# ChaissonLab/LRA

Measured on AMD Instinct MI355X. Metric: aligned Gbp/s, 30 kb ONT vs GRCh38 (MapRead_lowacc end to end incl. SAM text), per job, higher is better.
Workload: dtype int32

## Files before the change

lra_amd/csrc/aog.hip:

```cpp
#include "common.h"
#include <stdlib.h>
#include <algorithm>
#include <vector>
#include <type_traits>

namespace {

constexpr int MISS = -(1 << 30);
enum { A_DONE = 0, A_LEFT = 1, A_DOWN = 2, A_DIAG = 3, A_BORDER = 4, A_GAPLEFT = 5, A_GAPDOWN = 6 };

constexpr int CLASS_A_BYTES = 10 * 1024;
constexpr int CLASS_B_BYTES = 64 * 1024;
constexpr int CLASS_M1_BYTES = 20 * 1024;
constexpr int CLASS_M2_BYTES = 32 * 1024;
constexpr int LN_MAX = 24, LN_ROWW = 2;
constexpr int LN_ARROW_WORDS = LN_MAX * LN_ROWW, LN_PREV_WORDS = LN_MAX + 2, LN_CODE_BYTES = LN_MAX + 1;
constexpr int LN_BYTES = 64 * (4 * LN_ARROW_WORDS + 4 * LN_PREV_WORDS + 2 * LN_CODE_BYTES);
constexpr int NCLS = 19;
constexpr int CLASS_S_BYTES = 2560;

__device__ __forceinline__ int code_n(unsigned char c) {
  if (c < 8) return c & 3;
  switch (c) {
    case 'A': case 'a': return 0;
    case 'C': case 'c': return 1;
    case 'G': case 'g': return 2;
    case 'T': case 't': return 3;
    default: return 4;
  }
}

struct Geo {
  int qLen, tLen, diag, k, R, qB, tB;
  bool top;
  int n;
  int nUsed;
};

__device__ __forceinline__ bool make_geo(int qLen, int tLen, int k0, Geo& g) {
  g.qLen = qLen; g.tLen = tLen;
  g.diag = max(1, min(qLen, tLen));
  int k = min(g.diag, k0);
  g.top = true;
  if (g.diag + 2 * k >= max(qLen, tLen)) { k *= 2; g.top = false; }
  g.k = k;
  g.R = 2 * k + 3;
  long n = (long)(3 + k + g.diag) * g.R;
  g.qB = min(g.diag + k, qLen + 1);
  g.tB = min(g.diag + k, tLen + 1);
  if (n > (1L << 28)) { g.n = 0; g.nUsed = 0; return false; }
  g.n = (int)n;
  g.nUsed = g.top ? g.n : min(g.n, g.tB * g.R);
  return true;
}

__host__ __device__ __forceinline__ long align4(long x) { return (x + 3) & ~3L; }

__device__ __forceinline__ long need_bytes(const Geo& g) {
  long suf = g.top ? (4L * g.n + align4(g.n)) : 0;
  return 4L * g.nUsed + align4(g.nUsed) + suf + 16L * (g.diag + 1) + align4(g.qLen + 1) + align4(g.tLen + 1);
}

struct Work {
  int* sPre; int* sSuf; int* loMax; int* loIdx; int* upMax; int* upIdx;
  signed char* pPre; signed char* pSuf; unsigned char* qc; unsigned char* tc;
};

template <typename BytePtr>
__device__ __forceinline__ Work carve(BytePtr base, const Geo& g) {
  Work w;
  auto* p = base;
  w.sPre = (int*)p; p += 4L * g.nUsed;
  w.sSuf = (int*)p; if (g.top) p += 4L * g.n;
  w.loMax = (int*)p; p += 4L * (g.diag + 1);
  w.loIdx = (int*)p; p += 4L * (g.diag + 1);
  w.upMax = (int*)p; p += 4L * (g.diag + 1);
  w.upIdx = (int*)p; p += 4L * (g.diag + 1);
  w.pPre = (signed char*)p; p += align4(g.nUsed);
  w.pSuf = (signed char*)p; if (g.top) p += align4(g.n);
  w.qc = (unsigned char*)p; p += align4(g.qLen + 1);
  w.tc = (unsigned char*)p;
  return w;
}

__device__ __forceinline__ void wave_sync() {
  __builtin_amdgcn_fence(__ATOMIC_RELEASE, "workgroup");
  __builtin_amdgcn_wave_barrier();
  __builtin_amdgcn_fence(__ATOMIC_ACQUIRE, "workgroup");
}

__device__ __forceinline__ void wave_sync_lds() {
  __builtin_amdgcn_fence(__ATOMIC_RELEASE, "wavefront");
  __builtin_amdgcn_wave_barrier();
  __builtin_amdgcn_fence(__ATOMIC_ACQUIRE, "wavefront");
}

struct Problem {
  const char* q; const char* t;
  int qLen, tLen, k0, m, mm, indel;
};

__device__ __forceinline__ int dpp_from_prev_lane(int v) { return __builtin_amdgcn_update_dpp(MISS, v, 0x138, 0xf, 0xf, false); }
__device__ __forceinline__ int dpp_from_next_lane(int v) { return __builtin_amdgcn_update_dpp(MISS, v, 0x130, 0xf, 0xf, false); }

template <int G, typename ArrowPtr, typename CodePtr>
__device__ __forceinline__ int reg_fill(int lane, int gbase, const Geo& g, int m, int mm, int indel, ArrowPtr P, CodePtr qc, CodePtr tc) {
  const int qLen = g.qLen, tLen = g.tLen, k = g.k, R = g.R, diag = g.diag, qB = g.qB, tB = g.tB;
  auto pre = [&](int i, int j) -> int {
    int v = MISS;
    if (j == 0 && i >= 1 && i < k + 1) v = indel * i;
    if (i == 0 && j >= 1 && j <= k + 1) v = indel * j;
    if (i == 0 && j == 0) v = 0;
    if (qLen >= tLen) { if (j == i + k + 1 && i <= diag - k - 1) v = MISS; if (i == j + k + 1 && j >= 1 && j < diag + k - 1) v = MISS; }
    if (qLen <= tLen) { if (i == j + k + 1 && j < diag - 1) v = MISS; if (j == i + k + 1 && j >= 1 && j < diag + k) v = MISS; }
    return v;
  };
  const int Wd = 2 * k + 3;
  const int sLast = max((qB - 1) + (tB - 1), 0);
  const int ci = qB - 1, cj = tB - 1;
  int vE = MISS, vO = MISS;
  const bool firstE = ((0 - k - 1) & 1) == 0;
  const int dE = 2 * lane - k - 1, dO = dE + 1;
  const bool okE = 2 * lane < Wd && dE >= -k && dE <= k, okO = 2 * lane + 1 < Wd && dO >= -k && dO <= k;
  const int sLoE = okE ? 2 + abs(dE) : INT_MAX, sHiE = min(2 * (qB - 1) - dE, 2 * (tB - 1) + dE);
  const int sLoO = okO ? 2 + abs(dO) : INT_MAX, sHiO = min(2 * (qB - 1) - dO, 2 * (tB - 1) + dO);
  const int s0E = firstE ? 0 : 1, s0O = firstE ? 1 : 0;
  int iE = (s0E + dE) >> 1, jE = s0E - iE, iO = (s0O + dO) >> 1, jO = s0O - iO;
  int adE = jE * R + 2 * lane, adO = jO * R + 2 * lane + 1;
  auto codes_match = [&](int i, int j) -> bool { return qc[min(max(i, 0), qLen)] == tc[min(max(j, 0), tLen)]; };
  bool eqE = codes_match(iE, jE), eqO = codes_match(iO, jO);
  auto step = [&](int s, auto isE) {
    constexpr bool E = decltype(isE)::value;
    const int nb1 = E ? dpp_from_prev_lane(vO) : dpp_from_next_lane(vE);
    const int i = E ? iE : iO, j = E ? jE : jO;
    const bool nxt = codes_match(i + 1, j + 1);
    int v = MISS;
    if (s >= (E ? sLoE : sLoO) && s <= (E ? sHiE : sHiO)) {
      const int sIns = (E ? nb1 : vE) + indel;
      const int sDel = (E ? vO : nb1) + indel;
      const int sMat = (E ? vE : vO) + ((E ? eqE : eqO) ? m : mm);
      const int best = max(sIns, max(sDel, sMat));
      v = best;
      P[E ? adE : adO] = (signed char)((best == sIns) ? A_LEFT : (best == sDel) ? A_DOWN : A_DIAG);
    } else if (s <= k + 1) {
      if (2 * lane + (E ? 0 : 1) < Wd && i >= 0 && j >= 0) v = pre(i, j);
    }
    if (E) { vE = v; eqE = nxt; iE++; jE++; adE += R; } else { vO = v; eqO = nxt; iO++; jO++; adO += R; }
  };
  int s = 0;
  bool lastE;
  if (firstE) {
    for (; s + 1 <= sLast; s += 2) { step(s, std::true_type{}); step(s + 1, std::false_type{}); }
    lastE = false;
    if (s <= sLast) { step(s, std::true_type{}); lastE = true; }
  } else {
    for (; s + 1 <= sLast; s += 2) { step(s, std::false_type{}); step(s + 1, std::true_type{}); }
    lastE = true;
    if (s <= sLast) { step(s, std::false_type{}); lastE = false; }
  }
  const int ddc = ci - cj + k + 1;
  const int corner = lastE ? vE : vO;
  return (ci >= 0 && cj >= 0 && ddc >= 0 && ddc < Wd && ((ddc & 1) == 0) == lastE) ? __shfl(corner, gbase + (ddc >> 1)) : MISS;
}

template <int G, typename BytePtr>
__device__ __forceinline__ void solve(int wlane, const Problem& pr, const Geo& g, BytePtr mem, int* out_score,
                      int* out_nb, int* blocks, long cap, int* out_status, int* roll = nullptr, int chunkBytes = 8192) {
  const int qLen = g.qLen, tLen = g.tLen, k = g.k, R = g.R, diag = g.diag, n = g.n, nUsed = g.nUsed;
  const int m = pr.m, mm = pr.mm, indel = pr.indel;
  const int lane = wlane & (G - 1), gbase = wlane - lane;
  Work w = carve(mem, g);
  int status = 0;
  auto PI = [&](int i, int j) { return j * R + (i - j) + k + 1; };
  auto inb = [&](int s) { return s >= 0 && s < n; };
#define PSET(slot, sc, ar)                                                         \
  do { int s__ = (slot); if (inb(s__)) { if (s__ < nUsed) { if (!rolling) w.sPre[s__] = (sc); w.pPre[s__] = (ar); } } else status |= LRA_ST_OOB_SLOT; } while (0)
#define SSET(slot, sc, ar)                                                         \
  do { int s__ = (slot); if (inb(s__)) { w.sSuf[s__] = (sc); w.pSuf[s__] = (ar); } else status |= LRA_ST_OOB_SLOT; } while (0)

  for (int x = lane; x <= qLen; x += G) w.qc[x] = x ? code_n((unsigned char)pr.q[x - 1]) : 0;
  for (int x = lane; x <= tLen; x += G) w.tc[x] = x ? code_n((unsigned char)pr.t[x - 1]) : 0;
  const bool codesInLds = qLen + tLen + 2 <= 4096;
  const bool rolling = roll != nullptr && !g.top && (k + 2 <= G || (2 * k + 3 <= 256 && codesInLds));
  unsigned char* lq = (unsigned char*)(roll + 768); unsigned char* lt = lq + (qLen + 1);
  if (rolling && codesInLds) {
    for (int x = lane; x <= qLen; x += G) lq[x] = x ? code_n((unsigned char)pr.q[x - 1]) : 0;
    for (int x = lane; x <= tLen; x += G) lt[x] = x ? code_n((unsigned char)pr.t[x - 1]) : 0;
  }
  if (rolling) {
    const long head = min((long)nUsed, (long)((16 - ((uintptr_t)&w.pPre[0] & 15)) & 15));
    for (long x = lane; x < head; x += G) w.pPre[x] = -1;
    const long body = (nUsed - head) >> 4;
    int4* p16 = (int4*)(&w.pPre[0] + head);
    for (long x = lane; x < body; x += G) p16[x] = make_int4(-1, -1, -1, -1);
    for (long x = head + (body << 4) + lane; x < nUsed; x += G) w.pPre[x] = -1;
  }
  else for (int x = lane; x < nUsed; x += G) { w.sPre[x] = MISS; w.pPre[x] = -1; }
  if (g.top)
    for (int x = lane; x < n; x += G) { w.sSuf[x] = MISS; w.pSuf[x] = -1; }
  for (int x = lane; x <= diag; x += G) { w.loMax[x] = MISS; w.loIdx[x] = 0; w.upMax[x] = MISS; w.upIdx[x] = 0; }
  wave_sync();
  for (int i = 1 + lane; i < k + 1; i += G) PSET(PI(i, 0), indel * i, A_LEFT);
  for (int j = 1 + lane; j <= k + 1; j += G) PSET(PI(0, j), indel * j, A_DOWN);
  if (lane == 0) PSET(PI(0, 0), 0, A_DONE);
  wave_sync();
  if (qLen >= tLen) {
    for (int i = lane; i <= diag - k - 1; i += G) PSET(PI(i, i + k + 1), MISS, A_BORDER);
    for (int i = 1 + lane; i < diag + k - 1; i += G) PSET(PI(i + k + 1, i), MISS, A_BORDER);
  }
  if (qLen <= tLen) {
    for (int j = lane; j < diag - 1; j += G) PSET(PI(j + k + 1, j), MISS, A_BORDER);
    for (int j = 1 + lane; j < diag + k; j += G) PSET(PI(j - k - 1, j), MISS, A_BORDER);
  }
  wave_sync();
  const int qB = g.qB, tB = g.tB;
  int rollResult = MISS;
  if (rolling) {
    auto pre = [&](int i, int j) -> int {
      int v = MISS;
      if (j == 0 && i >= 1 && i < k + 1) v = indel * i;
      if (i == 0 && j >= 1 && j <= k + 1) v = indel * j;
      if (i == 0 && j == 0) v = 0;
      if (qLen >= tLen) { if (j == i + k + 1 && i <= diag - k - 1) v = MISS; if (i == j + k + 1 && j >= 1 && j < diag + k - 1) v = MISS; }
      if (qLen <= tLen) { if (i == j + k + 1 && j < diag - 1) v = MISS; if (j == i + k + 1 && j >= 1 && j < diag + k) v = MISS; }
      return v;
    };
    const int Wd = 2 * k + 3;
    const int sLast = (qB - 1) + (tB - 1);
    const bool inRegs = k + 2 <= G;
    if (inRegs) rollResult = codesInLds ? reg_fill<G>(lane, gbase, g, m, mm, indel, w.pPre, lq, lt) : reg_fill<G>(lane, gbase, g, m, mm, indel, w.pPre, w.qc, w.tc);
    for (int s = 0; !inRegs && s <= max(sLast, 0); s++) {
      int* cur = roll + (s % 3) * 256; const int* p1 = roll + ((s + 2) % 3) * 256; const int* p2 = roll + ((s + 1) % 3) * 256;
      int jlo = max(1, max(s - qB + 1, (s - k + 1) >> 1));
      if (s - k < 0) jlo = max(1, s - qB + 1);
      const int jhi = min(tB - 1, min(s - 1, (s + k) >> 1));
      for (int dd = lane; dd < Wd; dd += G) {
        const int d = dd - k - 1;
        int v = MISS;
        if (((s + d) & 1) == 0) {
          const int i = (s + d) >> 1, j = s - i;
          if (i >= 0 && j >= 0) {
            if (s >= 2 && j >= jlo && j <= jhi && d >= -k && d <= k) {
              const int sIns = p1[dd - 1] + indel, sDel = p1[dd + 1] + indel;
              const int sMat = p2[dd] + (lq[i] == lt[j] ? m : mm);
              const int best = max(sIns, max(sDel, sMat));
              const int ar = (best == sIns) ? A_LEFT : (best == sDel) ? A_DOWN : A_DIAG;
              v = best;
              w.pPre[PI(i, j)] = (signed char)ar;
            } else v = pre(i, j);
            if (i == qB - 1 && j == tB - 1) rollResult = v;
          }
        }
        cur[dd] = v;
      }
      wave_sync_lds();
    }
    wave_sync();
    if (!inRegs) { const int ddc = (qB - 1) - (tB - 1) + k + 1; rollResult = (ddc >= 0 && ddc < Wd) ? __shfl(rollResult, gbase + (ddc % G)) : MISS; }
  }
  for (int s = 2; !rolling && s <= (qB - 1) + (tB - 1); s++) {
    int jlo = max(1, max(s - qB + 1, (s - k + 1) >> 1));
    if (s - k < 0) jlo = max(1, s - qB + 1);
    int jhi = min(tB - 1, min(s - 1, (s + k) >> 1));
    for (int j = jlo + lane; j <= jhi; j += G) {
      int i = s - j;
      int sIns = w.sPre[PI(i - 1, j)] + indel;
      int sDel = w.sPre[PI(i, j - 1)] + indel;
      int sMat = w.sPre[PI(i - 1, j - 1)] + (w.qc[i] == w.tc[j] ? m : mm);
      int best = max(sIns, max(sDel, sMat));
      int ar = (best == sIns) ? A_LEFT : (best == sDel) ? A_DOWN : A_DIAG;
      int slot = PI(i, j);
      w.sPre[slot] = best;
      w.pPre[slot] = (signed char)ar;
    }
    wave_sync();
  }

  int ti, tj;
  int result;
  long nb = 0;
  const long iter_cap = 4L * (qLen + tLen + 8);
  int run = 0;
  auto flush = [&](int i_after, int j_after) {
    if (run > 0) {
      if (nb < cap) { blocks[3 * nb] = i_after; blocks[3 * nb + 1] = j_after; blocks[3 * nb + 2] = run; }
      else status |= LRA_ST_CAPACITY;
      nb++;
      run = 0;
    }
  };

  if (g.top) {
    for (int j = 1 + lane; j < tB && j <= diag; j += G) {
      int bm = MISS, bi = 0;
      int ihi = min(qB, j + k + 1);
      for (int i = max(1, j - k); i < ihi && i < qLen - k; i++) {
        int v = w.sPre[PI(i, j)];
        if (v >= bm) { bm = v; bi = i; }
      }
      w.loMax[j] = bm; w.loIdx[j] = bi;
    }
    for (int i = 1 + lane; i <= diag && i < qB; i += G) {
      int bm = MISS, bj = 0;
      int jhi = min(tB - 1, i + k);
      for (int j = max(1, i - k); j <= jhi && j < tLen; j++) {
        int v = w.sPre[PI(i, j)];
        if (v > bm) { bm = v; bj = j; }
      }
      w.upMax[i] = bm; w.upIdx[i] = bj;
    }
    if (lane == 0) {
      if (qLen >= tLen) { w.loMax[0] = 0; w.loIdx[0] = 0; }
      if (qLen <= tLen) { w.upMax[0] = 0; w.upIdx[0] = 0; }
    }
    wave_sync();
    const int qStart = max(0, qLen - diag);
    const int tStart = max(0, tLen - diag);
    const int tLow = max(0, tLen - diag - k - 1 - 1);
    const int qLow = max(0, qLen - diag - k - 1);
    const int tEnd = tLen + 1;
    auto SI = [&](int ii, int jj) {
      int a = ii - qLow, b = jj - tLow;
      return b * R + (a - b) + k + 1;
    };
    if (qLen >= tLen) {
      for (int i = qLow + lane; i < qStart + k + 1; i += G) SSET(SI(i, 0), w.loMax[0], A_GAPLEFT);
      wave_sync();
      for (int j = 1 + lane; j <= diag; j += G) SSET(SI(qLow + j - 1, j), w.loMax[j], A_GAPLEFT);
      wave_sync();
      for (int j = tStart + 1 + lane; j < tEnd - k; j += G) SSET(SI(qStart + (j - tStart - 1) + k + 1, j), MISS, A_BORDER);
      wave_sync();
    }
    if (qLen <= tLen) {
      for (int j = tLow + lane; j < tStart + k + 2; j += G) SSET(SI(qStart, j), w.upMax[0], A_GAPDOWN);
      wave_sync();
      for (int j = tStart + 1 + lane; j < tEnd; j += G) {
        int i = qStart + 1 + (j - tStart - 1);
        SSET(SI(i, j - k - 1), (i <= diag ? w.upMax[i] : MISS), A_GAPDOWN);
      }
      wave_sync();
      for (int j = tStart + lane; j < tEnd - k - 1; j += G) SSET(SI(qStart + (j - tStart), j + k + 1), MISS, A_BORDER);
      wave_sync();
    }
    const int c0 = qStart + diag - tLen;
    const bool qLong = qLen >= tLen;
    for (int s = (qLow + 1) + (tLow + 1); s <= qLen + tLen; s++) {
      int num = s - c0 - k;
      int jlo = (num >= 0) ? ((num + 1) >> 1) : -((-num) >> 1);
      jlo = max(jlo, max(tLow + 1, s - qLen));
      int num2 = s - c0 + k;
      int jhi = (num2 >= 0) ? (num2 >> 1) : -((-num2 + 1) >> 1);
      jhi = min(jhi, min(tLen, s - qLow - 1));
      for (int j = jlo + lane; j <= jhi; j += G) {
        int i = s - j;
        int delClose = MISS, insClose = MISS;
        if (qLong) delClose = (j <= diag) ? w.loMax[j] : MISS;
        else insClose = (i <= diag) ? w.upMax[i] : MISS;
        int a = SI(i - 1, j), b = SI(i, j - 1), c = SI(i - 1, j - 1);
        if (!inb(a) || !inb(b) || !inb(c)) { status |= LRA_ST_OOB_SLOT; continue; }
        int sIns = w.sSuf[a] + indel;
        int sDel = w.sSuf[b] + indel;
        int sMat = w.sSuf[c] + (w.qc[i] == w.tc[j] ? m : mm);
        int best = max(delClose, max(insClose, max(sIns, max(sDel, sMat))));
        int ar = (best == sIns) ? A_LEFT : (best == sDel) ? A_DOWN : (best == sMat) ? A_DIAG
                 : (best == delClose) ? A_GAPLEFT : A_GAPDOWN;
        SSET(SI(i, j), best, (signed char)ar);
      }
      wave_sync();
    }
    ti = qLen; tj = tLen;
    int s0 = SI(ti, tj);
    int arrow = inb(s0) ? w.pSuf[s0] : -1;
    result = inb(s0) ? w.sSuf[s0] : MISS;
    if (lane == 0) {
      long it = 0;
      while (arrow != A_DONE && arrow != A_GAPDOWN && arrow != A_GAPLEFT && ti >= 0 && tj >= 0) {
        if (++it > iter_cap) { status |= LRA_ST_NO_TERMINATION; break; }
        if (arrow == A_DIAG) { run++; ti--; tj--; }
        else if (arrow == A_LEFT) { flush(ti, tj); ti--; }
        else if (arrow == A_DOWN) { flush(ti, tj); tj--; }
        else { status |= LRA_ST_NO_TERMINATION; break; }
        if (ti >= 0 && tj >= 0) { int sl = SI(ti, tj); arrow = inb(sl) ? w.pSuf[sl] : -1; if (!inb(sl)) status |= LRA_ST_OOB_SLOT; }
      }
      flush(ti, tj);
      if (arrow == A_GAPDOWN && ti >= 0 && ti <= diag) tj = w.upIdx[ti];
      else if (arrow == A_GAPLEFT && tj >= 0 && tj <= diag) ti = w.loIdx[tj];
    }
  } else {
    ti = qB - 1; tj = tB - 1;
    result = rolling ? rollResult : w.sPre[PI(ti, tj)];
  }
  if (rolling) {
    unsigned char* chunk = (unsigned char*)(roll + 768 + 1024);
    const int chRows = max(1, chunkBytes / R);
    int cLo = 1, cHi = 0;
    auto arrowAt = [&](int i, int j) -> int {
      if (j < cLo || j > cHi) {
        cHi = j; cLo = max(0, j - chRows + 1);
        wave_sync();
        const long base = (long)cLo * R, len = (long)(cHi - cLo + 1) * R;
        for (long x = lane; x < len; x += G) chunk[x] = (unsigned char)w.pPre[base + x];
        wave_sync();
      }
      return (int)(signed char)chunk[(j - cLo) * R + (i - j) + k + 1];
    };
    auto flushL = [&](int i_after, int j_after) {
      if (run > 0) {
        if (nb < cap) { if (lane == 0) { blocks[3 * nb] = i_after; blocks[3 * nb + 1] = j_after; blocks[3 * nb + 2] = run; } }
        else status |= LRA_ST_CAPACITY;
        nb++;
        run = 0;
      }
    };
    constexpr int A_OFF = 100, A_WIN = 101;
    const unsigned long long gmask = (~0ULL >> (64 - G)) << gbase;
    if (ti >= 0 && tj >= 0 && inb(PI(ti, tj))) {
      while (true) {
        (void)arrowAt(ti, tj);
        const int jl = tj - lane;
        const bool on = ti - lane >= 0 && jl >= 0;
        const int a = !on ? A_OFF : jl < cLo ? A_WIN : (int)(signed char)chunk[(jl - cLo) * R + (ti - tj) + k + 1];
        const unsigned long long nd = (__ballot(a != A_DIAG) & gmask) >> gbase;
        const int f = nd ? __ffsll((long long)nd) - 1 : G;
        run += f; ti -= f; tj -= f;
        if (f == G) { if (ti < 0 || tj < 0) break; continue; }
        const int af = __shfl(a, gbase + f);
        if (af == A_WIN) continue;
        if (af == A_OFF) break;
        if (af == A_LEFT) { flushL(ti, tj); ti--; }
        else if (af == A_DOWN) { flushL(ti, tj); tj--; }
        else { if (af != A_BORDER && af != A_DONE && af != A_GAPLEFT && af != A_GAPDOWN) status |= LRA_ST_NO_TERMINATION; break; }
        if (ti < 0 || tj < 0) break;
      }
    }
    flushL(ti, tj);
  } else if (lane == 0) {
    int arrow = (ti >= 0 && tj >= 0 && inb(PI(ti, tj))) ? w.pPre[PI(ti, tj)] : A_DONE;
    long it = 0;
    while (arrow != A_BORDER && arrow != A_DONE && ti >= 0 && tj >= 0) {
      if (++it > iter_cap) { status |= LRA_ST_NO_TERMINATION; break; }
      if (arrow == A_DIAG) { run++; ti--; tj--; }
      else if (arrow == A_LEFT) { flush(ti, tj); ti--; }
      else if (arrow == A_DOWN) { flush(ti, tj); tj--; }
      else { if (arrow != A_GAPLEFT && arrow != A_GAPDOWN) status |= LRA_ST_NO_TERMINATION; break; }
      if (ti < 0 || tj < 0) break;
      arrow = w.pPre[PI(ti, tj)];
    }
    flush(ti, tj);
  }
#undef PSET
#undef SSET
  nb = __shfl(nb, gbase);
  int fi = __shfl(ti, gbase), fj = __shfl(tj, gbase);
  wave_sync();
  long nw = min(nb, cap);
  for (long x = lane; x < (nw + 1) / 2; x += G) {
    long y = nw - 1 - x;
    int a0 = blocks[3 * x], a1 = blocks[3 * x + 1], a2 = blocks[3 * x + 2];
    int b0 = blocks[3 * y], b1 = blocks[3 * y + 1], b2 = blocks[3 * y + 2];
    blocks[3 * x] = b0 - fi; blocks[3 * x + 1] = b1 - fj; blocks[3 * x + 2] = b2;
    if (y != x) { blocks[3 * y] = a0 - fi; blocks[3 * y + 1] = a1 - fj; blocks[3 * y + 2] = a2; }
  }
  for (int off = G / 2; off > 0; off >>= 1) status |= __shfl_xor(status, off);
  if (lane == 0) {
    int r = result;
    if (r < -(1 << 29)) r = (int)(unsigned int)((long)INT_MIN + ((long)r - (long)MISS));
    *out_score = r;
    *out_nb = (int)nb;
    *out_status = status;
  }
}

template <int G, typename BytePtr>
__device__ __forceinline__ void solve_reg(int wlane, const Problem& pr, const Geo& g, BytePtr mem, int* out_score, int* out_nb, int* blocks, long cap, int* out_status) {
  const int qLen = g.qLen, tLen = g.tLen, k = g.k, R = g.R, diag = g.diag, n = g.n, nUsed = g.nUsed;
  const int m = pr.m, mm = pr.mm, indel = pr.indel;
  const int lane = wlane & (G - 1), gbase = wlane - lane;
  auto* P = (signed char*)&mem[0];
  auto* qc = (unsigned char*)&mem[align4(nUsed)];
  auto* tc = (unsigned char*)&mem[align4(nUsed) + align4(qLen + 1)];
  int status = 0;
  auto PI = [&](int i, int j) { return j * R + (i - j) + k + 1; };
  auto inb = [&](int s_) { return s_ >= 0 && s_ < n; };
#define PSETA(slot, ar) do { int s__ = (slot); if (inb(s__)) { if (s__ < nUsed) P[s__] = (ar); } else status |= LRA_ST_OOB_SLOT; } while (0)
  for (int x = lane; x <= qLen; x += G) qc[x] = x ? code_n((unsigned char)pr.q[x - 1]) : 0;
  for (int x = lane; x <= tLen; x += G) tc[x] = x ? code_n((unsigned char)pr.t[x - 1]) : 0;
  { auto* P4 = (int*)&mem[0]; for (int x = lane; x < (int)(align4(nUsed) >> 2); x += G) P4[x] = -1; }
  wave_sync();
  for (int i = 1 + lane; i < k + 1; i += G) PSETA(PI(i, 0), A_LEFT);
  for (int j = 1 + lane; j <= k + 1; j += G) PSETA(PI(0, j), A_DOWN);
  if (lane == 0) PSETA(PI(0, 0), A_DONE);
  wave_sync();
  if (qLen >= tLen) {
    for (int i = lane; i <= diag - k - 1; i += G) PSETA(PI(i, i + k + 1), A_BORDER);
    for (int i = 1 + lane; i < diag + k - 1; i += G) PSETA(PI(i + k + 1, i), A_BORDER);
  }
  if (qLen <= tLen) {
    for (int j = lane; j < diag - 1; j += G) PSETA(PI(j + k + 1, j), A_BORDER);
    for (int j = 1 + lane; j < diag + k; j += G) PSETA(PI(j - k - 1, j), A_BORDER);
  }
  wave_sync();
#undef PSETA
  const int qB = g.qB, tB = g.tB;
  const int result = reg_fill<G>(lane, gbase, g, m, mm, indel, P, qc, tc);
  wave_sync();
  int ti = qB - 1, tj = tB - 1;
  long nb = 0; int run = 0;
  auto flushL = [&](int i_after, int j_after) {
    if (run > 0) {
      if (nb < cap) { if (lane == 0) { blocks[3 * nb] = i_after; blocks[3 * nb + 1] = j_after; blocks[3 * nb + 2] = run; } }
      else status |= LRA_ST_CAPACITY;
      nb++;
      run = 0;
    }
  };
  constexpr int A_OFF = 100;
  const unsigned long long gmask = (~0ULL >> (64 - G)) << gbase;
  if (ti >= 0 && tj >= 0 && inb(PI(ti, tj))) {
    while (true) {
      const bool on = ti - lane >= 0 && tj - lane >= 0;
      const int a = on ? (int)P[PI(ti, tj) - lane * R] : A_OFF;
      const unsigned long long nd = (__ballot(a != A_DIAG) & gmask) >> gbase;
      const int f = nd ? __ffsll((long long)nd) - 1 : G;
      run += f; ti -= f; tj -= f;
      if (f == G) { if (ti < 0 || tj < 0) break; continue; }
      const int af = __shfl(a, gbase + f);
      if (af == A_OFF) break;
      if (af == A_LEFT) { flushL(ti, tj); ti--; }
      else if (af == A_DOWN) { flushL(ti, tj); tj--; }
      else { if (af != A_BORDER && af != A_DONE && af != A_GAPLEFT && af != A_GAPDOWN) status |= LRA_ST_NO_TERMINATION; break; }
      if (ti < 0 || tj < 0) break;
    }
  }
  flushL(ti, tj);
  wave_sync();
  const long nw = min(nb, cap);
  for (long x = lane; x < (nw + 1) / 2; x += G) {
    const long y = nw - 1 - x;
    const int a0 = blocks[3 * x], a1 = blocks[3 * x + 1], a2 = blocks[3 * x + 2];
    const int b0 = blocks[3 * y], b1 = blocks[3 * y + 1], b2 = blocks[3 * y + 2];
    blocks[3 * x] = b0 - ti; blocks[3 * x + 1] = b1 - tj; blocks[3 * x + 2] = b2;
    if (y != x) { blocks[3 * y] = a0 - ti; blocks[3 * y + 1] = a1 - tj; blocks[3 * y + 2] = a2; }
  }
  for (int off = G / 2; off > 0; off >>= 1) status |= __shfl_xor(status, off);
  if (lane == 0) {
    int r = result;
    if (r < -(1 << 29)) r = (int)(unsigned int)((long)INT_MIN + ((long)r - (long)MISS));
    *out_score = r;
    *out_nb = (int)nb;
    *out_status = status;
  }
}
__device__ __forceinline__ long need_bytes_reg(const Geo& g) { return align4(g.nUsed) + align4(g.qLen + 1) + align4(g.tLen + 1); }
constexpr int REG_S_BYTES = 2048, REG_M_BYTES = 8192, REG_L_BYTES = 32768;
constexpr int REG_L_USED = 16384;

struct BatchArgs {
  int n;
  const char* qseq; const char* tseq;
  const uint64_t* q_off; const int32_t* q_len; const uint64_t* t_off; const int32_t* t_len;
  const int32_t* k;
  int m, mm, indel;
  int32_t* score; int32_t* nblocks; int32_t* blocks; const uint64_t* block_off; int32_t* status;
  int* counts; int* offs; int* cursor; unsigned char* cls8; int* list;
  char* gscratch; long gslot_bytes; int gslots;
  char* gscratchB; long gslotB_bytes; int gslotsB;
  int chunk_bytes;
};

__device__ __forceinline__ bool load_problem(const BatchArgs& a, int p, Problem& pr, Geo& g, int& range_ok) {
  pr.q = a.qseq + a.q_off[p]; pr.t = a.tseq + a.t_off[p];
  pr.qLen = a.q_len[p]; pr.tLen = a.t_len[p]; pr.k0 = a.k[p];
  pr.m = a.m; pr.mm = a.mm; pr.indel = a.indel;
  bool ok = pr.qLen >= 0 && pr.tLen >= 0 && pr.k0 >= 1 && make_geo(pr.qLen, pr.tLen, pr.k0, g);
  long mx = max(abs(a.m), max(abs(a.mm), abs(a.indel)));
  range_ok = ok && ((long)(pr.qLen + pr.tLen + 16) * (mx + 1) < (1L << 28));
  return range_ok;
}

constexpr int CLS_ITEMS = 16;
// ... 132 lines not shown
  constexpr int LN_ARROW_WORDS = LN_MAX * LN_ROWW, LN_PREV_WORDS = LN_MAX + 2, LN_CODE_BYTES = LN_MAX + 1;
  constexpr int LN_BYTES = 64 * (4 * LN_ARROW_WORDS + 4 * LN_PREV_WORDS + 2 * LN_CODE_BYTES);
  __shared__ __attribute__((aligned(16))) char smem[LN_BYTES];
  const int lane = threadIdx.x;
  unsigned* AR = (unsigned*)smem;
  int* PV = (int*)(smem + 64 * 4 * LN_ARROW_WORDS);
  unsigned char* QC = (unsigned char*)(smem + 64 * 4 * (LN_ARROW_WORDS + LN_PREV_WORDS));
  unsigned char* TC = QC + 64 * LN_CODE_BYTES;
  const int count = a.counts[cls];
  for (int x0 = blockIdx.x * 64; x0 < count; x0 += gridDim.x * 64) {
    const int x = x0 + lane;
    if (x < count) {
      const int p = a.list[a.offs[cls] + x];
      Problem pr; Geo g; int ok;
      load_problem(a, p, pr, g, ok);
      const int qLen = g.qLen, tLen = g.tLen, k = g.k, diag = g.diag, qB = g.qB, tB = g.tB;
      const int m = pr.m, mm = pr.mm, indel = pr.indel;
      {
        unsigned char cq[LN_MAX], ct[LN_MAX];
#pragma unroll
        for (int i = 0; i < LN_MAX; i++) { cq[i] = i < qLen ? (unsigned char)pr.q[i] : 0; ct[i] = i < tLen ? (unsigned char)pr.t[i] : 0; }
#pragma unroll
        for (int i = 0; i < LN_MAX; i++) { QC[(i + 1) * 64 + lane] = (unsigned char)code_n(cq[i]); TC[(i + 1) * 64 + lane] = (unsigned char)code_n(ct[i]); }
      }
      auto in_region = [&](int i, int j) { return i >= 1 && i <= qB - 1 && j >= 1 && j <= tB - 1 && i - j <= k && j - i <= k; };
      auto pre = [&](int i, int j) -> int {
        int v = MISS;
        if (j == 0 && i >= 1 && i < k + 1) v = indel * i;
        if (i == 0 && j >= 1 && j <= k + 1) v = indel * j;
        if (i == 0 && j == 0) v = 0;
        if (qLen >= tLen) { if (j == i + k + 1 && i <= diag - k - 1) v = MISS; if (i == j + k + 1 && j >= 1 && j < diag + k - 1) v = MISS; }
        if (qLen <= tLen) { if (i == j + k + 1 && j < diag - 1) v = MISS; if (j == i + k + 1 && j >= 1 && j < diag + k) v = MISS; }
        return v;
      };
      auto pre_arrow = [&](int i, int j) -> int {
        int v = -1;
        if (i < 0 || j < 0) return v;
        if (j == 0 && i >= 1 && i < k + 1) v = A_LEFT;
        if (i == 0 && j >= 1 && j <= k + 1) v = A_DOWN;
        if (i == 0 && j == 0) v = A_DONE;
        if (qLen >= tLen) { if (j == i + k + 1 && i <= diag - k - 1) v = A_BORDER; if (i == j + k + 1 && j >= 1 && j < diag + k - 1) v = A_BORDER; }
        if (qLen <= tLen) { if (i == j + k + 1 && j < diag - 1) v = A_BORDER; if (j == i + k + 1 && j >= 1 && j < diag + k) v = A_BORDER; }
        return v;
      };
      for (int j = 1; j <= tB - 1; j++) {
        const int ilo = max(1, j - k), ihi = min(qB - 1, j + k);
        const int tcj = TC[j * 64 + lane];
        int left = pre(ilo - 1, j);
        int dg = in_region(ilo - 1, j - 1) ? PV[(ilo - 1) * 64 + lane] : pre(ilo - 1, j - 1);
        unsigned long long acc = 0;
        const int hi2 = j >= 2 ? min(qB - 1, j - 1 + k) : 0;
        for (int i = ilo; i <= ihi; i++) {
          int up;
          if (i <= hi2) up = PV[i * 64 + lane];
          else up = (j == 1 && i < k + 1) ? indel * i : MISS;
          const int sIns = left + indel, sDel = up + indel, sMat = dg + (QC[i * 64 + lane] == tcj ? m : mm);
          const int best = max(sIns, max(sDel, sMat));
          const int ar = (best == sIns) ? A_LEFT : (best == sDel) ? A_DOWN : A_DIAG;
          acc |= (unsigned long long)ar << (2 * (i - ilo));
          PV[i * 64 + lane] = best;
          dg = up; left = best;
        }
        AR[((j - 1) * LN_ROWW) * 64 + lane] = (unsigned)acc; if (LN_ROWW > 1) AR[((j - 1) * LN_ROWW + 1) * 64 + lane] = (unsigned)(acc >> 32);
      }
      const int ci = qB - 1, cj = tB - 1;
      const int result = in_region(ci, cj) ? PV[ci * 64 + lane] : ((ci >= 0 && cj >= 0) ? pre(ci, cj) : MISS);
      auto arrow_at = [&](int i, int j) -> int {
        if (!in_region(i, j)) return pre_arrow(i, j);
        const int sh = 2 * (i - max(1, j - k));
        const unsigned w = AR[((j - 1) * LN_ROWW + (LN_ROWW > 1 ? (sh >> 5) : 0)) * 64 + lane];
        return (int)((w >> (sh & 31)) & 3u);
      };
      const long cap = (long)(a.block_off[p + 1] - a.block_off[p]);
      int* blocks = a.blocks + 3 * a.block_off[p];
      int status = 0;
      long nb = 0; int fi = ci, fj = cj;
      for (int pass = 0; pass < 2; pass++) {
        const long nw = min(nb, cap);
        long w = 0; int run = 0; int ti = ci, tj = cj;
        auto flush = [&](int i_after, int j_after) {
          if (run > 0) {
            if (pass == 1 && w < nw) { int* b = blocks + 3 * (nw - 1 - w); b[0] = i_after - fi; b[1] = j_after - fj; b[2] = run; }
            w++; run = 0;
          }
        };
        int arrow = (ti >= 0 && tj >= 0) ? arrow_at(ti, tj) : A_DONE;
        while (arrow != A_BORDER && arrow != A_DONE && ti >= 0 && tj >= 0) {
          if (arrow == A_DIAG) { run++; ti--; tj--; }
          else if (arrow == A_LEFT) { flush(ti, tj); ti--; }
          else if (arrow == A_DOWN) { flush(ti, tj); tj--; }
          else { if (arrow != A_GAPLEFT && arrow != A_GAPDOWN) status |= LRA_ST_NO_TERMINATION; break; }
          if (ti < 0 || tj < 0) break;
          arrow = arrow_at(ti, tj);
        }
        flush(ti, tj);
        if (pass == 0) { nb = w; fi = ti; fj = tj; if (nb > cap) status |= LRA_ST_CAPACITY; }
      }
      int r = result;
      if (r < -(1 << 29)) r = (int)(unsigned int)((long)INT_MIN + ((long)r - (long)MISS));
      a.score[p] = r; a.nblocks[p] = (int)nb; a.status[p] = status;
    }
  }
}

}

int lra_aog_launch_device(lra_ctx* ctx, int n, const char* d_qseq, const char* d_tseq, const uint64_t* d_q_off,
                          const int32_t* d_q_len, const uint64_t* d_t_off, const int32_t* d_t_len, const int32_t* d_k,
                          int m, int mm, int indel, int32_t* d_score, int32_t* d_nblocks, int32_t* d_blocks,
                          const uint64_t* d_block_off, int32_t* d_status) {
  if (!ctx) return LRA_ERR_INVALID;
  if (n < 0) return lra_set_err(ctx, LRA_ERR_INVALID, "n < 0");
  if (n == 0) return LRA_OK;
  LRA_HIP_CHECK(ctx, hipSetDevice(ctx->device));
  BatchArgs a;
  a.n = n; a.qseq = d_qseq; a.tseq = d_tseq; a.q_off = d_q_off; a.q_len = d_q_len; a.t_off = d_t_off; a.t_len = d_t_len;
  a.k = d_k; a.m = m; a.mm = mm; a.indel = indel;
  a.score = d_score; a.nblocks = d_nblocks; a.blocks = d_blocks; a.block_off = d_block_off; a.status = d_status;
  char* s0 = (char*)lra_scratch(ctx, 0, 384 + sizeof(int) * (size_t)n + (size_t)n + 64);
  if (!s0) return LRA_ERR_NOMEM;
  a.counts = (int*)s0; a.offs = a.counts + 32; a.cursor = a.counts + 64; a.list = (int*)(s0 + 384); a.cls8 = (unsigned char*)(a.list + n);
  const int perCu = ctx->pipelined ? 6 : 8;
  a.gslots = ctx->num_cu * perCu; a.gslot_bytes = 4L << 20;
  a.chunk_bytes = 8192;
  a.gslotsB = ctx->num_cu; a.gslotB_bytes = 8L << 20;
  a.gscratch = (char*)lra_scratch(ctx, 1, (size_t)a.gslots * a.gslot_bytes + (size_t)a.gslotsB * a.gslotB_bytes);
  if (!a.gscratch) return LRA_ERR_NOMEM;
  a.gscratchB = a.gscratch + (size_t)a.gslots * a.gslot_bytes;
  if (getenv("LRA_AOG_DBG")) {
    std::vector<int32_t> hq(n), ht(n), hk(n);
    (void)hipMemcpy(hq.data(), d_q_len, (size_t)n * 4, hipMemcpyDeviceToHost); (void)hipMemcpy(ht.data(), d_t_len, (size_t)n * 4, hipMemcpyDeviceToHost);
    (void)hipMemcpy(hk.data(), d_k, (size_t)n * 4, hipMemcpyDeviceToHost);
    long nTop = 0, nBigK = 0, steps = 0; long byNeed[8] = {0, 0, 0, 0, 0, 0, 0, 0}; long byK[4] = {0, 0, 0, 0}; long cellsBy[8] = {0, 0, 0, 0, 0, 0, 0, 0};
    for (int p = 0; p < n; p++) {
      const int q = hq[p], t = ht[p]; const int diag = std::max(1, std::min(q, t)); int k = std::min(diag, hk[p]); bool top = true;
      if (diag + 2 * k >= std::max(q, t)) { k *= 2; top = false; }
      const long R = 2 * k + 3, tB = std::min(diag + k, t + 1); const long nU = top ? (3 + k + diag) * R : std::min((3 + k + diag) * R, tB * R);
      if (top) { nTop++; continue; }
      if (k > 62) { nBigK++; continue; }
      const long need = nU + q + t + 8;
      const int b = need <= 2048 ? 0 : need <= 4096 ? 1 : need <= 8192 ? 2 : need <= 16384 ? 3 : need <= 32768 ? 4 : need <= 65536 ? 5 : need <= 160 * 1024 ? 6 : 7;
      byNeed[b]++; cellsBy[b] += nU; steps += q + t;
      byK[k <= 14 ? 0 : k <= 30 ? 1 : k <= 62 ? 2 : 3]++;
    }
    fprintf(stderr, "[aog] n %d top %ld k>62 %ld | arrows+codes <=2K %ld <=4K %ld <=8K %ld <=16K %ld <=32K %ld <=64K %ld <=160K %ld more %ld | cells(M) %.1f %.1f %.1f %.1f %.1f %.1f %.1f %.1f | k<=14 %ld <=30 %ld <=62 %ld | steps(M) %.1f\n",
            n, nTop, nBigK, byNeed[0], byNeed[1], byNeed[2], byNeed[3], byNeed[4], byNeed[5], byNeed[6], byNeed[7], cellsBy[0] / 1e6, cellsBy[1] / 1e6, cellsBy[2] / 1e6, cellsBy[3] / 1e6,
            cellsBy[4] / 1e6, cellsBy[5] / 1e6, cellsBy[6] / 1e6, cellsBy[7] / 1e6, byK[0], byK[1], byK[2], steps / 1e6);
  }
  LRA_HIP_CHECK(ctx, hipMemsetAsync(a.counts, 0, 384, ctx->stream));
  const int cblocks = (int)(((long)n + CLS_ITEMS * 1024 - 1) / (CLS_ITEMS * 1024));
  hipLaunchKernelGGL(aog_classify, dim3(cblocks), dim3(1024), 0, ctx->stream, a);
  hipLaunchKernelGGL(aog_offsets, dim3(1), dim3(64), 0, ctx->stream, a);
  hipLaunchKernelGGL(aog_scatter, dim3(cblocks), dim3(1024), 0, ctx->stream, a);
  int wgA = min((n + 3) / 4, ctx->num_cu * 5);
  int wgB = min(n, ctx->num_cu * 2);
  int wgC = min(n, a.gslots);
  LRA_HIP_CHECK(ctx, hipFuncSetAttribute((const void*)aog_kernel<7>, hipFuncAttributeMaxDynamicSharedMemorySize, 8 * CLASS_A_BYTES));
  LRA_HIP_CHECK(ctx, hipFuncSetAttribute((const void*)aog_kernel<1>, hipFuncAttributeMaxDynamicSharedMemorySize, CLASS_B_BYTES));
  LRA_HIP_CHECK(ctx, hipFuncSetAttribute((const void*)aog_kernel<9>, hipFuncAttributeMaxDynamicSharedMemorySize, 2 * CLASS_M2_BYTES));
  const hipStream_t sm = ctx->stream;
  const hipStream_t s1 = lra_side_fork(ctx, 1), s2 = lra_side_fork(ctx, 2), s3 = lra_side_fork(ctx, 3);
  lra_time_begin(ctx, "aog_lds_large", s1);
  hipLaunchKernelGGL(aog_kernel<1>, dim3(wgB), dim3(64), CLASS_B_BYTES, s1, a);
  lra_time_end(ctx, s1);
  lra_time_begin(ctx, "aog_lds_small", s2);
  hipLaunchKernelGGL(aog_kernel<7>, dim3(min((n + 7) / 8, ctx->num_cu * 2)), dim3(256), 8 * CLASS_A_BYTES, s2, a);
  hipLaunchKernelGGL(aog_kernel<0>, dim3(wgA), dim3(256), 4 * CLASS_A_BYTES, s2, a);
  lra_time_end(ctx, s2);
  lra_time_begin(ctx, "aog_lds_tiny", s2);
  hipLaunchKernelGGL(aog_kernel<3>, dim3(min((n + 15) / 16, ctx->num_cu * 8)), dim3(256), 16 * CLASS_S_BYTES, s2, a);
  lra_time_end(ctx, s2);
  lra_time_begin(ctx, "aog_lds_medium", s3);
  hipLaunchKernelGGL(aog_kernel<8>, dim3(min((n + 1) / 2, ctx->num_cu * 4)), dim3(64), 2 * CLASS_M1_BYTES, s3, a);
  hipLaunchKernelGGL(aog_kernel<9>, dim3(min((n + 1) / 2, ctx->num_cu * 2)), dim3(64), 2 * CLASS_M2_BYTES, s3, a);
  hipLaunchKernelGGL(aog_kernel<4>, dim3(min(n, ctx->num_cu * 8)), dim3(64), CLASS_M1_BYTES, s3, a);
  hipLaunchKernelGGL(aog_kernel<5>, dim3(min(n, ctx->num_cu * 5)), dim3(64), CLASS_M2_BYTES, s3, a);
  lra_time_end(ctx, s3);
  lra_time_begin(ctx, "aog_lane");
  const int nb64 = (n + 63) / 64;
  hipLaunchKernelGGL(aog_lane_kernel<24>, dim3(min(nb64, ctx->num_cu * 7)), dim3(64), 0, sm, a, 18);
  hipLaunchKernelGGL(aog_lane_kernel<16>, dim3(min(nb64, ctx->num_cu * 14)), dim3(64), 0, sm, a, 17);
  hipLaunchKernelGGL(aog_lane_kernel<10>, dim3(min(nb64, ctx->num_cu * 22)), dim3(64), 0, sm, a, 16);
  hipLaunchKernelGGL(aog_lane_kernel<6>, dim3(min(nb64, ctx->num_cu * 32)), dim3(64), 0, sm, a, 15);
  hipLaunchKernelGGL(aog_lane_kernel<3>, dim3(min(nb64, ctx->num_cu * 32)), dim3(64), 0, sm, a, 14);
  lra_time_end(ctx);
  lra_time_begin(ctx, "aog_reg");
  hipLaunchKernelGGL(aog_reg_kernel<10>, dim3(min((n + 15) / 16, ctx->num_cu * 10)), dim3(256), 16 * REG_S_BYTES, sm, a);
  lra_time_end(ctx);
  lra_time_begin(ctx, "aog_reg_medium", s2);
  hipLaunchKernelGGL(aog_reg_kernel<11>, dim3(min((n + 3) / 4, ctx->num_cu * 10)), dim3(128), 4 * REG_M_BYTES, s2, a);
  lra_time_end(ctx, s2);
  lra_time_begin(ctx, "aog_reg_large", s3);
  hipLaunchKernelGGL(aog_reg_kernel<12>, dim3(min(n, ctx->num_cu * 10)), dim3(64), REG_L_USED, s3, a);
  lra_time_end(ctx, s3);
  lra_time_begin(ctx, "aog_hbm");
  hipLaunchKernelGGL(aog_kernel<2>, dim3(wgC), dim3(64), (3 * 256 + 1024) * 4 + a.chunk_bytes, sm, a);
  hipLaunchKernelGGL(aog_kernel<6>, dim3(min(n, a.gslotsB)), dim3(64), (3 * 256 + 1024) * 4 + a.chunk_bytes, sm, a);
  lra_time_end(ctx);
  lra_side_join(ctx, 1); lra_side_join(ctx, 2); lra_side_join(ctx, 3);
  LRA_HIP_CHECK(ctx, hipGetLastError());
  return LRA_OK;
}

extern "C" int lra_affine_one_gap_align_batch(lra_ctx* ctx, int n, const char* d_qseq, const char* d_tseq,
                                              const uint64_t* d_q_off, const int32_t* d_q_len,
                                              const uint64_t* d_t_off, const int32_t* d_t_len,
                                              const int32_t* d_k, int m, int mm, int indel,
                                              int32_t* d_score, int32_t* d_nblocks, int32_t* d_blocks,
                                              const uint64_t* d_block_off, int32_t* d_status) {
  return lra_aog_launch_device(ctx, n, d_qseq, d_tseq, d_q_off, d_q_len, d_t_off, d_t_len, d_k, m, mm, indel, d_score, d_nblocks,
                               d_blocks, d_block_off, d_status);
}
```

Baseline: 1.066.

## Add register-wavefront fill and ballot traceback for two-band top alignment problems

Extends the DPP register anti-diagonal fill to the two-band (top) alignment case, storing scores and arrows for both the prefix and a new suffix sweep that folds in gap-close maxima. Traceback for these problems uses a wave-wide ballot to skip runs of diagonal arrows instead of a single-lane walk. Codes and gap maxima are staged in LDS when room allows. It replaces the per-antidiagonal loops with their wave syncs, at the cost of more code and register pressure. An env-gated debug histogram is also added.

```diff
diff --git a/lra_amd/csrc/aog.hip b/lra_amd/csrc/aog.hip
--- a/lra_amd/csrc/aog.hip
+++ b/lra_amd/csrc/aog.hip
@@ -103,8 +103,8 @@
 __device__ __forceinline__ int dpp_from_prev_lane(int v) { return __builtin_amdgcn_update_dpp(MISS, v, 0x138, 0xf, 0xf, false); }
 __device__ __forceinline__ int dpp_from_next_lane(int v) { return __builtin_amdgcn_update_dpp(MISS, v, 0x130, 0xf, 0xf, false); }
 
-template <int G, typename ArrowPtr, typename CodePtr>
-__device__ __forceinline__ int reg_fill(int lane, int gbase, const Geo& g, int m, int mm, int indel, ArrowPtr P, CodePtr qc, CodePtr tc) {
+template <int G, bool STORE = false, typename ArrowPtr, typename CodePtr>
+__device__ __forceinline__ int reg_fill(int lane, int gbase, const Geo& g, int m, int mm, int indel, ArrowPtr P, CodePtr qc, CodePtr tc, int* S = nullptr) {
   const int qLen = g.qLen, tLen = g.tLen, k = g.k, R = g.R, diag = g.diag, qB = g.qB, tB = g.tB;
   auto pre = [&](int i, int j) -> int {
     int v = MISS;
@@ -142,6 +142,7 @@
       const int best = max(sIns, max(sDel, sMat));
       v = best;
       P[E ? adE : adO] = (signed char)((best == sIns) ? A_LEFT : (best == sDel) ? A_DOWN : A_DIAG);
+      if (STORE) S[E ? adE : adO] = best;
     } else if (s <= k + 1) {
       if (2 * lane + (E ? 0 : 1) < Wd && i >= 0 && j >= 0) v = pre(i, j);
     }
@@ -161,6 +162,63 @@
   const int ddc = ci - cj + k + 1;
   const int corner = lastE ? vE : vO;
   return (ci >= 0 && cj >= 0 && ddc >= 0 && ddc < Wd && ((ddc & 1) == 0) == lastE) ? __shfl(corner, gbase + (ddc >> 1)) : MISS;
+}
+
+template <int G, typename ArrowPtr, typename CodePtr>
+__device__ __forceinline__ void reg_fill_suf(int lane, const Geo& g, int m, int mm, int indel, ArrowPtr P, int* S, CodePtr qc, CodePtr tc, const int* mx,
+                                             int qLow, int tLow, int c0) {
+  const int qLen = g.qLen, tLen = g.tLen, k = g.k, R = g.R, diag = g.diag;
+  const bool qLong = qLen >= tLen;
+  const int Wd = 2 * k + 3;
+  const int sBeg = qLow + tLow, sEnd = qLen + tLen;
+  const bool firstE = ((sBeg + c0 - k - 1) & 1) == 0;
+  const int eE = 2 * lane - k - 1, eO = eE + 1;
+  const int dE = eE + c0, dO = eO + c0;
+  auto sRange = [&](int dd, int e, int d, int& lo, int& hi) {
+    lo = INT_MAX; hi = INT_MIN;
+    if (dd < Wd && e >= -k && e <= k) { lo = 2 * max(tLow + 1, qLow + 1 - d) + d; hi = 2 * min(tLen, qLen - d) + d; }
+  };
+  int sLoE, sHiE, sLoO, sHiO;
+  sRange(2 * lane, eE, dE, sLoE, sHiE); sRange(2 * lane + 1, eO, dO, sLoO, sHiO);
+  const int s0E = firstE ? sBeg : sBeg + 1, s0O = firstE ? sBeg + 1 : sBeg;
+  int iE = (s0E + dE) >> 1, jE = s0E - iE, iO = (s0O + dO) >> 1, jO = s0O - iO;
+  auto SI = [&](int ii, int jj) { return (jj - tLow) * R + (ii - qLow - (jj - tLow)) + k + 1; };
+  int adE = SI(iE, jE), adO = SI(iO, jO);
+  auto codes_match = [&](int i, int j) -> bool { return qc[min(max(i, 0), qLen)] == tc[min(max(j, 0), tLen)]; };
+  auto mx_at = [&](int e, int i, int j) -> int { return mx[min(max(qLong ? (e == k + 1 ? j + 1 : j) : i, 0), diag)]; };
+  int vE = MISS, vO = MISS;
+  bool eqE = codes_match(iE, jE), eqO = codes_match(iO, jO);
+  int xE = mx_at(eE, iE, jE), xO = mx_at(eO, iO, jO);
+  auto step = [&](int s, auto isE) {
+    constexpr bool E = decltype(isE)::value;
+    const int nb1 = E ? dpp_from_prev_lane(vO) : dpp_from_next_lane(vE);
+    const int i = E ? iE : iO, j = E ? jE : jO, e = E ? eE : eO, x = E ? xE : xO;
+    const bool nxt = codes_match(i + 1, j + 1);
+    const int nx = mx_at(e, i + 1, j + 1);
+    int v;
+    if (s >= (E ? sLoE : sLoO) && s <= (E ? sHiE : sHiO)) {
+      const int sIns = (E ? nb1 : vE) + indel;
+      const int sDel = (E ? vO : nb1) + indel;
+      const int sMat = (E ? vE : vO) + ((E ? eqE : eqO) ? m : mm);
+      const int delClose = qLong ? x : MISS, insClose = qLong ? MISS : x;
+      const int best = max(delClose, max(insClose, max(sIns, max(sDel, sMat))));
+      const int ar = (best == sIns) ? A_LEFT : (best == sDel) ? A_DOWN : (best == sMat) ? A_DIAG : (best == delClose) ? A_GAPLEFT : A_GAPDOWN;
+      v = best;
+      const int ad = E ? adE : adO;
+      S[ad] = best; P[ad] = (signed char)ar;
+    } else {
+      v = (e == k + 1 || (e >= -k && e <= k && (qLong ? j == 0 : i == 0))) ? x : MISS;
+    }
+    if (E) { vE = v; eqE = nxt; xE = nx; iE++; jE++; adE += R; } else { vO = v; eqO = nxt; xO = nx; iO++; jO++; adO += R; }
+  };
+  int s = sBeg;
+  if (firstE) {
+    for (; s + 1 <= sEnd; s += 2) { step(s, std::true_type{}); step(s + 1, std::false_type{}); }
+    if (s <= sEnd) step(s, std::true_type{});
+  } else {
+    for (; s + 1 <= sEnd; s += 2) { step(s, std::false_type{}); step(s + 1, std::true_type{}); }
+    if (s <= sEnd) step(s, std::false_type{});
+  }
 }
 
 template <int G, typename BytePtr>
@@ -183,7 +241,9 @@
   const bool codesInLds = qLen + tLen + 2 <= 4096;
   const bool rolling = roll != nullptr && !g.top && (k + 2 <= G || (2 * k + 3 <= 256 && codesInLds));
   unsigned char* lq = (unsigned char*)(roll + 768); unsigned char* lt = lq + (qLen + 1);
-  if (rolling && codesInLds) {
+  const bool regTop = g.top && k + 2 <= G && min(qLen, tLen) >= 1 && (roll == nullptr || (codesInLds && (diag + 1) * 4 <= chunkBytes));
+  const bool codesLds = roll != nullptr && codesInLds && (rolling || regTop);
+  if (codesLds) {
     for (int x = lane; x <= qLen; x += G) lq[x] = x ? code_n((unsigned char)pr.q[x - 1]) : 0;
     for (int x = lane; x <= tLen; x += G) lt[x] = x ? code_n((unsigned char)pr.t[x - 1]) : 0;
   }
@@ -258,7 +318,12 @@
     wave_sync();
     if (!inRegs) { const int ddc = (qB - 1) - (tB - 1) + k + 1; rollResult = (ddc >= 0 && ddc < Wd) ? __shfl(rollResult, gbase + (ddc % G)) : MISS; }
   }
-  for (int s = 2; !rolling && s <= (qB - 1) + (tB - 1); s++) {
+  const unsigned char* cq = codesLds ? lq : w.qc; const unsigned char* ct = codesLds ? lt : w.tc;
+  if (regTop) {
+    reg_fill<G, true>(lane, gbase, g, m, mm, indel, w.pPre, cq, ct, w.sPre);
+    wave_sync();
+  }
+  for (int s = 2; !rolling && !regTop && s <= (qB - 1) + (tB - 1); s++) {
     int jlo = max(1, max(s - qB + 1, (s - k + 1) >> 1));
     if (s - k < 0) jlo = max(1, s - qB + 1);
     int jhi = min(tB - 1, min(s - 1, (s + k) >> 1));
@@ -284,6 +349,14 @@
   auto flush = [&](int i_after, int j_after) {
     if (run > 0) {
       if (nb < cap) { blocks[3 * nb] = i_after; blocks[3 * nb + 1] = j_after; blocks[3 * nb + 2] = run; }
+      else status |= LRA_ST_CAPACITY;
+      nb++;
+      run = 0;
+    }
+  };
+  auto flushL = [&](int i_after, int j_after) {
+    if (run > 0) {
+      if (nb < cap) { if (lane == 0) { blocks[3 * nb] = i_after; blocks[3 * nb + 1] = j_after; blocks[3 * nb + 2] = run; } }
       else status |= LRA_ST_CAPACITY;
       nb++;
       run = 0;
@@ -344,7 +417,18 @@
     }
     const int c0 = qStart + diag - tLen;
     const bool qLong = qLen >= tLen;
-    for (int s = (qLow + 1) + (tLow + 1); s <= qLen + tLen; s++) {
+    if (regTop) {
+      const int* mx = qLong ? w.loMax : w.upMax;
+      if (roll != nullptr) {
+        int* lmx = roll + 768 + 1024;
+        for (int x = lane; x <= diag; x += G) lmx[x] = mx[x];
+        wave_sync();
+        mx = lmx;
+      }
+      reg_fill_suf<G>(lane, g, m, mm, indel, w.pSuf, w.sSuf, cq, ct, mx, qLow, tLow, c0);
+      wave_sync();
+    }
+    for (int s = (qLow + 1) + (tLow + 1); !regTop && s <= qLen + tLen; s++) {
       int num = s - c0 - k;
       int jlo = (num >= 0) ? ((num + 1) >> 1) : -((-num) >> 1);
       jlo = max(jlo, max(tLow + 1, s - qLen));
@@ -372,7 +456,30 @@
     int s0 = SI(ti, tj);
     int arrow = inb(s0) ? w.pSuf[s0] : -1;
     result = inb(s0) ? w.sSuf[s0] : MISS;
-    if (lane == 0) {
+    if (regTop) {
+      constexpr int A_OFF = 100, A_OOB = 101;
+      const unsigned long long gmask = (~0ULL >> (64 - G)) << gbase;
+      if (arrow == -1) status |= LRA_ST_NO_TERMINATION;
+      while (arrow != -1 && arrow != A_DONE && arrow != A_GAPDOWN && arrow != A_GAPLEFT) {
+        const int sl = SI(ti, tj) - lane * R;
+        const int a = !(ti - lane >= 0 && tj - lane >= 0) ? A_OFF : !inb(sl) ? A_OOB : (int)w.pSuf[sl];
+        const unsigned long long nd = (__ballot(a != A_DIAG) & gmask) >> gbase;
+        const int f = nd ? __ffsll((long long)nd) - 1 : G;
+        run += f; ti -= f; tj -= f;
+        if (f == G) { arrow = A_DIAG; if (ti < 0 || tj < 0) break; continue; }
+        const int af = __shfl(a, gbase + f);
+        if (af == A_OFF) { arrow = A_DIAG; break; }
+        if (af == A_OOB) { status |= LRA_ST_OOB_SLOT | LRA_ST_NO_TERMINATION; arrow = -1; break; }
+        arrow = af;
+        if (af == A_LEFT) { flushL(ti, tj); ti--; }
+        else if (af == A_DOWN) { flushL(ti, tj); tj--; }
+        else { if (af != A_DONE && af != A_GAPDOWN && af != A_GAPLEFT) status |= LRA_ST_NO_TERMINATION; break; }
+        if (ti < 0 || tj < 0) break;
+      }
+      flushL(ti, tj);
+      if (arrow == A_GAPDOWN && ti >= 0 && ti <= diag) tj = w.upIdx[ti];
+      else if (arrow == A_GAPLEFT && tj >= 0 && tj <= diag) ti = w.loIdx[tj];
+    } else if (lane == 0) {
       long it = 0;
       while (arrow != A_DONE && arrow != A_GAPDOWN && arrow != A_GAPLEFT && ti >= 0 && tj >= 0) {
         if (++it > iter_cap) { status |= LRA_ST_NO_TERMINATION; break; }
@@ -403,14 +510,6 @@
         wave_sync();
       }
       return (int)(signed char)chunk[(j - cLo) * R + (i - j) + k + 1];
-    };
-    auto flushL = [&](int i_after, int j_after) {
-      if (run > 0) {
-        if (nb < cap) { if (lane == 0) { blocks[3 * nb] = i_after; blocks[3 * nb + 1] = j_after; blocks[3 * nb + 2] = run; } }
-        else status |= LRA_ST_CAPACITY;
-        nb++;
-        run = 0;
-      }
     };
     constexpr int A_OFF = 100, A_WIN = 101;
     const unsigned long long gmask = (~0ULL >> (64 - G)) << gbase;
@@ -426,6 +525,26 @@
         if (f == G) { if (ti < 0 || tj < 0) break; continue; }
         const int af = __shfl(a, gbase + f);
         if (af == A_WIN) continue;
+        if (af == A_OFF) break;
+        if (af == A_LEFT) { flushL(ti, tj); ti--; }
+        else if (af == A_DOWN) { flushL(ti, tj); tj--; }
+        else { if (af != A_BORDER && af != A_DONE && af != A_GAPLEFT && af != A_GAPDOWN) status |= LRA_ST_NO_TERMINATION; break; }
+        if (ti < 0 || tj < 0) break;
+      }
+    }
+    flushL(ti, tj);
+  } else if (regTop) {
+    constexpr int A_OFF = 100;
+    const unsigned long long gmask = (~0ULL >> (64 - G)) << gbase;
+    if (ti >= 0 && tj >= 0 && inb(PI(ti, tj))) {
+      while (true) {
+        const bool on = ti - lane >= 0 && tj - lane >= 0;
+        const int a = on ? (int)w.pPre[PI(ti, tj) - lane * R] : A_OFF;
+        const unsigned long long nd = (__ballot(a != A_DIAG) & gmask) >> gbase;
+        const int f = nd ? __ffsll((long long)nd) - 1 : G;
+        run += f; ti -= f; tj -= f;
+        if (f == G) { if (ti < 0 || tj < 0) break; continue; }
+        const int af = __shfl(a, gbase + f);
         if (af == A_OFF) break;
         if (af == A_LEFT) { flushL(ti, tj); ti--; }
         else if (af == A_DOWN) { flushL(ti, tj); tj--; }
@@ -864,6 +983,27 @@
   hipLaunchKernelGGL(aog_classify, dim3(cblocks), dim3(1024), 0, ctx->stream, a);
   hipLaunchKernelGGL(aog_offsets, dim3(1), dim3(64), 0, ctx->stream, a);
   hipLaunchKernelGGL(aog_scatter, dim3(cblocks), dim3(1024), 0, ctx->stream, a);
+  if (getenv("LRA_AOG_DBG")) {
+    std::vector<int32_t> hq(n), ht(n), hk(n); std::vector<unsigned char> hc(n);
+    (void)hipStreamSynchronize(ctx->stream);
+    (void)hipMemcpy(hq.data(), d_q_len, (size_t)n * 4, hipMemcpyDeviceToHost); (void)hipMemcpy(ht.data(), d_t_len, (size_t)n * 4, hipMemcpyDeviceToHost);
+    (void)hipMemcpy(hk.data(), d_k, (size_t)n * 4, hipMemcpyDeviceToHost); (void)hipMemcpy(hc.data(), a.cls8, (size_t)n, hipMemcpyDeviceToHost);
+    long cnt[NCLS] = {}, top[NCLS] = {}, topReg[NCLS] = {}, maxNeed[NCLS] = {}; double cPre[NCLS] = {}, cSuf[NCLS] = {}, arr[NCLS] = {};
+    for (int p = 0; p < n; p++) {
+      const int c = (int)(signed char)hc[p];
+      if (c < 0 || c >= NCLS || hk[p] < 1 || hq[p] < 0 || ht[p] < 0) continue;
+      const int q = hq[p], t = ht[p]; const int diag = std::max(1, std::min(q, t)); int k = std::min(diag, hk[p]); bool tp = true;
+      if (diag + 2 * k >= std::max(q, t)) { k *= 2; tp = false; }
+      const long R = 2 * k + 3, nn = (3L + k + diag) * R, tB = std::min(diag + k, t + 1), nU = tp ? nn : std::min(nn, tB * R);
+      const long need = 5 * nU + (tp ? 5 * nn : 0) + 16L * (diag + 1) + q + t + 8;
+      const int G = c == 3 ? 16 : (c >= 7 && c <= 9) ? 32 : 64;
+      cnt[c]++; top[c] += tp; topReg[c] += tp && k + 2 <= G && std::min(q, t) >= 1 && ((c != 2 && c != 6) || (q + t + 2 <= 4096 && (diag + 1) * 4 <= 8192)); maxNeed[c] = std::max(maxNeed[c], need);
+      cPre[c] += (double)std::max(tB - 1, 0L) * (2 * k + 1); if (tp) cSuf[c] += (double)diag * (2 * k + 1); arr[c] += nU + (tp ? nn : 0);
+    }
+    for (int c = 0; c < NCLS; c++)
+      if (cnt[c]) fprintf(stderr, "[aog] n %d class %d problems %ld two-band %ld (register sweep %ld) cells(M) prefix %.2f suffix %.2f arrows(MB) %.2f largest need(KB) %.1f\n",
+                          n, c, cnt[c], top[c], topReg[c], cPre[c] / 1e6, cSuf[c] / 1e6, arr[c] / 1e6, maxNeed[c] / 1024.0);
+  }
   int wgA = min((n + 3) / 4, ctx->num_cu * 5);
   int wgB = min(n, ctx->num_cu * 2);
   int wgC = min(n, a.gslots);
```

New measurement: 1.081 (median of 6 runs). 1.4% higher.
